# ACMEAtronOmatic/DSen2

Hardware: AMD Instinct MI355X
Metric: 32x32x6 patches/sec (DSen2_20, d=6, batch 512) (higher is better)
Workload: dtype f32; 1 GPU; DSen2_20 d=6 F=128 fp32, 512 synthetic 32x32 patches (4+6 bands) per GPU per step, he_uniform random-init weights; batch_per_gpu=512, parallelism=patch-sharded dp1, backend=rccl, output_gather=False

## Files before the change

dsen2_amd/asm_contract.py:

```python
import os
import re
import subprocess
import tempfile

HERE = os.path.dirname(os.path.abspath(__file__))
CSRC = os.path.join(HERE, 'csrc')
DMA_SOURCES = ['conv3x3_body32.hip', 'conv3x3_body16w.hip']


class AsmContractError(RuntimeError):
    pass


def _code_lines(text):
    return [ln.strip() for ln in text.splitlines() if ln.strip() and not ln.strip().startswith((';', '.', '//'))]


def _kernels(text):
    out, name, body = {}, None, []
    for ln in text.splitlines():
        m = re.match(r'^(_Z\w+):', ln)
        if m:
            name, body = m.group(1), []
            continue
# ... 6 lines not shown
                name = None
    return out


def normalised(body):
    return [re.sub(r'\.L\w+', 'L', re.sub(r'\s+', ' ', ln)) for ln in body]


def compile_isa(hipcc, flags, path, out, verbose=False):
    cmd = [hipcc] + [f for f in flags if f != '-fPIC'] + ['-S', '--cuda-device-only', path, '-o', out]
    if verbose:
        print(' '.join(cmd), flush=True)
    subprocess.check_call(cmd, stderr=subprocess.DEVNULL)
    with open(out) as f:
        return f.read()


def _needer(src):
    def need(cond, msg, ctx=()):
        if not cond:
            raise AsmContractError('%s: %s %s' % (src, msg, list(ctx)))
    return need


def check_listing(text, src):
    code = _code_lines(text)
    code = [ln.split(';')[0].strip() for ln in code]
    need = _needer(src)

    m0 = [i for i, ln in enumerate(code) if re.search(r'\bm0\b', ln)]
    need(m0, 'no M0 use found (the DMA statements are gone?)')
    dma = [i for i, ln in enumerate(code) if ln.startswith('buffer_load_dword') and ln.endswith('lds')]
    need(dma, 'no LDS-DMA instruction found')
    allowed = set()
    for i in dma:
        need(code[i - 1] == 's_nop 0' and re.match(r's_mov_b32 m0, (s\d+|vcc_lo|vcc_hi)$', code[i - 2]), 'DMA without its M0 write + wait state',
             code[i - 2:i + 1])
        allowed.update((i - 2,))
        for j in range(i - 3, max(i - 7, -1), -1):
            if re.match(r's_mov_b32 (s\d+|vcc_lo|vcc_hi), m0$', code[j]):
                allowed.add(j)
                break
        k = i + 1
        if re.match(r's_mov_b32 m0, (s\d+|vcc_lo|vcc_hi)$', code[k]):
            allowed.add(k)
    for i in m0:
        need(i in allowed, 'M0 touched outside a DMA statement', code[max(0, i - 2):i + 3])
    saves = sum(1 for ln in code if re.match(r's_mov_b32 (s\d+|vcc_lo|vcc_hi), m0$', ln))
    need(saves > 0, 'the DMA statements no longer save M0')
    STEP_MFMAS = 9 * 32
    need(not any(ln.startswith(('s_swappc', 's_call')) for ln in code), 'a DMA kernel calls a function (an epilogue was not inlined)')
    kernels = _kernels(text)
    need(kernels, 'no kernel found')
    n_dma_kernels = 0
    for name, body in kernels.items():
        if not any(ln.startswith('buffer_load_dword') and ln.endswith('lds') for ln in body):
            continue
        n_dma_kernels += 1
        chain = '_chain_kernel' in name
        if not chain:
            need(not any('scratch_' in ln for ln in body), 'kernel %s spills registers' % name)
        else:
            mf = [i for i, ln in enumerate(body) if ln.startswith('v_mfma')]
            need(mf and len(mf) % STEP_MFMAS == 0, 'chain kernel %s: %d MFMAs is not a whole number of item bodies' % (name, len(mf)))
            for g in range(0, len(mf), STEP_MFMAS):
                inner = body[mf[g]:mf[g + STEP_MFMAS - 1]]
                need(not any('scratch_' in ln for ln in inner), 'chain kernel %s spills inside an item body' % name)
            for i, ln in enumerate(body):
                if 'scratch_' not in ln:
                    continue
                nxt = None
                for ln2 in body[i + 1:]:
                    if ln2.startswith('v_mfma'):
                        break
                    mm = re.search(r'vmcnt\((\d+)\)', ln2) if ln2.startswith('s_waitcnt') else None
                    if mm:
                        nxt = int(mm.group(1))
                        break
                need(nxt == 0, 'chain kernel %s: scratch access outside a drained region (next vmcnt wait: %r)' % (name, nxt), [ln])
        back = [ln for ln in body[-40:] if ln.startswith('s_waitcnt') and 'vmcnt' in ln]
        need(back and back[-1].replace(' ', '') in ('s_waitcntvmcnt(0)', 's_waitcntvmcnt(0)lgkmcnt(0)'),
             'kernel %s does not drain its DMAs before s_endpgm' % name, back[-3:])
    need(n_dma_kernels > 0, 'no LDS-DMA kernel found')
    if src == 'conv3x3_body16w.hip':
        expect = {0: (0, 32), 1: (64, 64), 3: (64, 64)}
        expect3 = {0: (0, 64), 1: (64, 96), 3: (64, 64)}

        def count(pattern, want, msg, product=lambda m: True):
            found = []
            for name, body in kernels.items():
                m = re.search(pattern, name)
                if not m or not product(m):
                    continue
                found.append(body)
                loads = sum(1 for ln in body if ln.startswith('buffer_load_dwordx4') and not ln.endswith('lds'))
                stores = sum(1 for ln in body if ln.startswith('buffer_store_dwordx4'))
                need((loads, stores) == want(m), msg(m) % (loads, stores, want(m)))
            return found

        def total(e):
            return lambda m: (sum(v[0] for v in e.values()), sum(v[1] for v in e.values()))

        found = count(r'conv3x3_body16[wx]_kernelILi(\d+)ELi(\d+)ELi(\d+)ELi(\d+)E', lambda m: expect[int(m.group(3))],
                      lambda m: 'epilogue ' + m.group(3) + ' has %d loads / %d stores, the waits count %r', lambda m: int(m.group(4)) == 0)
        need(len(found) >= 6, 'expected the 6 product instantiations of the bf16 body kernel, found %d' % len(found))
        for body in found:
            other = [ln for ln in body if re.match(r'(buffer|global|flat)_(load|store|atomic)', ln)
                     and not ln.startswith(('buffer_load_dwordx4', 'buffer_store_dwordx4'))]
            need(len(other) <= 1, 'unexpected vector-memory instructions in the bf16 body kernel', other[:4])
        found3 = count(r'conv3x3_body16w_x3_kernelILi(\d+)ELi(\d+)ELi(\d+)E', lambda m: expect3[int(m.group(3))],
                       lambda m: 'bf16x3 epilogue ' + m.group(3) + ' has %d loads / %d stores, the waits count %r')
        need(len(found3) == 6, 'expected the 6 instantiations of the bf16x3 body kernel, found %d' % len(found3))
        chains = count(r'conv3x3_body16w_chain_kernelILi(\d+)ELi(\d+)ELi(\d+)E', total(expect),
                       lambda m: 'chain kernel has %d loads / %d stores in its epilogues, the waits count %r', lambda m: int(m.group(3)) == 0)
        need(len(chains) == 2, 'expected the 2 product instantiations of the chain kernel, found %d' % len(chains))
        chains3 = count(r'conv3x3_body16w_x3_chain_kernelILi(\d+)ELi(\d+)E', total(expect3),
                        lambda m: 'bf16x3 chain kernel has %d loads / %d stores in its epilogues, the waits count %r')
        need(len(chains3) == 2, 'expected the 2 instantiations of the bf16x3 chain kernel, found %d' % len(chains3))


def check_out_mfma_listing(text, src='conv3x3_out_mfma.hip'):
    need = _needer(src)
    kernels = {k: v for k, v in _kernels(text).items() if 'conv3x3_out_mfma_kernel' in k}
    need(len(kernels) == 4, 'expected 4 instantiations of the output kernel, found %d' % len(kernels))
    for name, body in kernels.items():
        need(not any('scratch_' in ln for ln in body), 'kernel %s spills registers' % name)
        need(not any(ln.startswith(('s_swappc', 's_call')) for ln in body), 'kernel %s calls a function' % name)
        mf = [i for i, ln in enumerate(body) if ln.startswith('v_mfma')]
        need(mf, 'kernel %s has no MFMA' % name)
        waits = [ln for ln in body[mf[0]:mf[-1]] if ln.startswith('s_waitcnt') and 'vmcnt' in ln]
        need(len(waits) >= 8, 'kernel %s: no operand waits between its MFMAs' % name)
        bad = [ln for ln in waits if int(re.search(r'vmcnt\((\d+)\)', ln).group(1)) < 8]
        need(not bad, 'kernel %s waits for the loads of the NEXT unit' % name, bad[:4])
    return True


def check_first16_listing(text, src='conv3x3_first16.hip'):
    need = _needer(src)
    kernels = {k: v for k, v in _kernels(text).items() if 'conv3x3_first16_kernel' in k}
    need(len(kernels) == 8, 'expected 8 instantiations of the kernel, found %d' % len(kernels))
    for name, body in kernels.items():
        need(not any('scratch_' in ln for ln in body), 'kernel %s spills registers' % name)
        need(not any(ln.startswith(('s_swappc', 's_call')) for ln in body), 'kernel %s calls a function' % name)
        stores = [ln for ln in body if ln.startswith('buffer_store_dwordx4')]
        need(stores, 'kernel %s has no 128-bit buffer store' % name)
        bad = [ln for ln in stores if not re.search(r'\], 0 offen', ln)]
        need(not bad, 'kernel %s: 128-bit buffer store with a register soffset (late data read, unpadded hazard)' % name, bad[:2])
        need(not any(ln.startswith('global_store') for ln in body), 'kernel %s stores outside its buffer descriptors' % name)
        mf = [i for i, ln in enumerate(body) if ln.startswith('v_mfma')]
        need(mf, 'kernel %s has no MFMA' % name)
        x3 = 'ELb1EEE' in name
        floor = 24 if x3 else 16
        loop = body[mf[0]:]
        scat = [i for i, ln in enumerate(loop) if ln.startswith('ds_write_b16')]
        need(scat, 'kernel %s: no halo scatter after the first MFMA' % name)
        waits = [ln for ln in loop[:scat[-1]] if ln.startswith('s_waitcnt') and 'vmcnt' in ln]
        low = [ln for ln in waits if int(re.search(r'vmcnt\((\d+)\)', ln).group(1)) < floor]
        need(not low, 'kernel %s: a wait inside the tile loop drains the deferred stores (divergent branch in the loop body?)' % name, low[:4])
    return True


TRAFFIC_KERNELS = {
    'dsen2_20_fp32': ('conv3x3_body32.hip', r'conv3x3_body32_kernelILi128ELi128ELi0ELi0ELi0ELb1ELb1E'),
    'vdsen2_20_bf16': ('conv3x3_body16w.hip', r'conv3x3_body16w_chain_kernelILi128ELi256ELi0E'),
    'dsen2_20_bf16x3': ('conv3x3_body16w.hip', r'conv3x3_body16w_x3_chain_kernelILi64ELi128E'),
    'vdsen2_20_fp32': ('conv3x3_body32.hip', r'conv3x3_body32_kernelILi256ELi256ELi0ELi0ELi0ELb1ELb1E'),
    'dsen2_20_bf16': ('conv3x3_body16w.hip', r'conv3x3_body16w_chain_kernelILi64ELi128ELi0E'),
    'vdsen2_20_bf16x3': ('conv3x3_body16w.hip', r'conv3x3_body16w_x3_chain_kernelILi128ELi256E'),
}
ISA_JSON = os.path.join(HERE, 'kernel_isa.json')


def isa_hashes(text):
    import hashlib
    out = {}
    for name, body in _kernels(text).items():
        out[name] = hashlib.sha256('\n'.join(normalised(body)).encode()).hexdigest()
    return out


def traffic_kernel_hashes(listings):
    out = {}
    for cfg, (src, pat) in TRAFFIC_KERNELS.items():
        hits = {k: v for k, v in isa_hashes(listings[src]).items() if re.search(pat, k)}
        if len(hits) != 1:
            raise AsmContractError('%s: expected one kernel matching %s, found %d' % (src, pat, len(hits)))
        (k, v), = hits.items()
        out[cfg] = {'kernel': k, 'isa_sha256': v}
    return out


def check_sources(hipcc, flags, verbose=False, isa_json=None):
    listings = {}
    with tempfile.TemporaryDirectory(prefix='dsen2_asm_') as tmp:
        for src in DMA_SOURCES + ['conv3x3_out_mfma.hip', 'conv3x3_first16.hip']:
            listings[src] = compile_isa(hipcc, flags, os.path.join(CSRC, src), os.path.join(tmp, src + '.s'), verbose)
            if src in DMA_SOURCES:
                check_listing(listings[src], src)
            elif src == 'conv3x3_first16.hip':
                check_first16_listing(listings[src], src)
            else:
                check_out_mfma_listing(listings[src], src)
    hashes = traffic_kernel_hashes(listings)
    if isa_json:
        import json
        with open(isa_json, 'w') as f:
            json.dump(hashes, f, indent=1, sort_keys=True)
            f.write('\n')
    return hashes
```

dsen2_amd/csrc/capi.hip:

```cpp

#include <chrono>
#include <cstdarg>
#include <cstdio>
#include <cstring>
#include <exception>
#include <new>
#include <vector>

#include "capi_internal.h"

using namespace dsen2;

namespace {

thread_local char g_err[512] = "";

#ifdef DSEN2_DIAG
Tuning g_diag_tuning;
unsigned long long* g_diag_stamps = nullptr;
#endif
Tuning default_tuning() {
#ifdef DSEN2_DIAG
  return g_diag_tuning;
#else
// ... 317 lines not shown
    off += align_up(floats);
    return p;
  };
  if (mask & ~1) {
    r.x10 = take(pix * m->c10);
    r.x20 = take(pix * m->c20);
    if (m->c60 > 0) r.x60 = take(pix * m->c60);
    r.y = take(pix * m->cout);
  }
  r.bytes = off * sizeof(float);
  return r;
}

static int check_ensemble_shape(const dsen2_model* m, int n, int h, int w, int mask) {
  if (mask <= 0 || mask > 255) return fail(DSEN2_ERR_INVALID, "ensemble mask %d outside 1..255", mask);
  if (int rc = check_shape(m, n, h, w)) return rc;
  if (int rc = check_shape(m, n, w, h)) return rc;
  int cmax = m->cout;
  for (int c : {m->c10, m->c20, m->c60}) cmax = c > cmax ? c : cmax;
  if ((size_t)n * h * w * cmax >= ((size_t)1 << 31))
    return fail(DSEN2_ERR_INVALID, "batch of %d images of %dx%d: a tensor of 2^31 elements or more", n, h, w);
  return DSEN2_OK;
}

static int forward_ensemble(dsen2_model* m, const float* x10, const float* x20, const float* x60, float* out, int n, int h, int w,
                            int mask, void* workspace, size_t workspace_bytes, void* stream_) {
  if (!m || !x10 || !x20 || !out || !workspace) return fail(DSEN2_ERR_INVALID, "NULL argument");
  if ((m->c60 > 0) != (x60 != nullptr)) return fail(DSEN2_ERR_INVALID, "x60 must be given iff the model has a 60 m input");
  if (mask <= 0 || mask > 255) return fail(DSEN2_ERR_INVALID, "ensemble mask %d outside 1..255", mask);
  if (n == 0) return DSEN2_OK;
  if (!m->loaded) return fail(DSEN2_ERR_NO_WEIGHTS, "dsen2_model_load_weights has not been called");
  if (int rc = check_ensemble_shape(m, n, h, w, mask)) return rc;
  if (int rc = check_device(m)) return rc;
  const size_t pix = (size_t)n * h * w;
  const float* const ins[3] = {x10, x20, x60};
  const int cs[3] = {m->c10, m->c20, m->c60};
  for (int k = 0; k < 3; ++k)
    if (ins[k] && overlaps(ins[k], pix * cs[k] * sizeof(float), out, pix * m->cout * sizeof(float)))
      return fail(DSEN2_ERR_INVALID, "the output aliases an input");
  const EnsembleWs E = ensemble_ws(m, n, h, w, mask, reinterpret_cast<char*>(workspace));
  if (workspace_bytes < E.bytes) return fail(DSEN2_ERR_WORKSPACE, "workspace %zu < %zu bytes", workspace_bytes, E.bytes);
  hipStream_t stream = (hipStream_t)stream_;
  int count = 0;
  for (int op = 0; op < 8; ++op) count += (mask >> op) & 1;
  int done = 0;
  for (int op = 0; op < 8; ++op) {
    if (!((mask >> op) & 1)) continue;
    const bool first = done == 0, last = done + 1 == count;
    if (op == 0) {
      const ForwardWs B = forward_ws(m, n, h, w, E.fwd);
      if (int rc = forward_launches(m, x10, x20, x60, out, n, h, w, B, 0, false, stream, nullptr)) return rc;
    } else {
      const bool tr = op & 1;
      const int th = tr ? w : h, tw = tr ? h : w;
      float* const turned[3] = {E.x10, E.x20, E.x60};
      for (int k = 0; k < 3; ++k)
        if (ins[k]) HIP_TRY(launch_dihedral(ins[k], turned[k], n, cs[k], h, w, op, nullptr, false, stream));
      const ForwardWs B = forward_ws(m, n, th, tw, E.fwd);
      if (int rc = forward_launches(m, E.x10, E.x20, E.x60, E.y, n, th, tw, B, 0, false, stream, nullptr)) return rc;
      if (first) HIP_TRY(launch_dihedral(E.y, out, n, m->cout, th, tw, op, nullptr, true, stream));
      else HIP_TRY(launch_dihedral_accumulate(E.y, out, n, m->cout, h, w, op, last ? count : 0, stream));
    }
    ++done;
  }
  return DSEN2_OK;
}

extern "C" {

const char* dsen2_version(void) {
#ifdef DSEN2_DIAG
  return "dsen2_hip 0.3-diag (gfx950; fp32 MFMA 32x32x2 / bf16 MFMA 16x16x32 / bf16x3; DIAGNOSTIC build)";
#else
  return "dsen2_hip 0.3 (gfx950; fp32 MFMA 32x32x2 / bf16 MFMA 16x16x32 / bf16x3)";
#endif
}
const char* dsen2_last_error(void) { return g_err; }

#ifdef DSEN2_DIAG
int dsen2_diag_set(int key, int value) {
  Tuning& t = g_diag_tuning;
  switch (key) {
    case 0:
      if (value != 0 && (value < 11 || value > 14)) return fail(DSEN2_ERR_INVALID, "body variant %d unknown", value);
      t.first = value == 0 ? FirstKernel::Tile16 : FirstKernel::Direct;
      t.body = value == 0 ? BodyKernel::Tile : BodyKernel::Body32;
      t.body32 = value == 0 ? Body32Form::DeferStagger : static_cast<Body32Form>(value - 11);
      return DSEN2_OK;
    case 2:
      if (value != 0 && value != 2 && value != 3) return fail(DSEN2_ERR_INVALID, "output variant %d unknown", value);
      t.out = value == 2 ? OutKernel::MfmaThenValu : value == 3 ? OutKernel::Valu : OutKernel::Tile;
      return DSEN2_OK;
    case 1: t.ablate = value; return DSEN2_OK;
    case 3: t.grid_cap = value; return DSEN2_OK;
    case 4: t.chain = value; return DSEN2_OK;
    case 5: t.first_ablate = value; return DSEN2_OK;
    case 6: t.out_ablate = value; return DSEN2_OK;
  }
  return fail(DSEN2_ERR_INVALID, "unknown diagnostic key %d", key);
}
int dsen2_diag_set_stamps(void* dev_buffer) {
  g_diag_stamps = reinterpret_cast<unsigned long long*>(dev_buffer);
  return DSEN2_OK;
}
#endif

int dsen2_device_count(void) {
  int n = 0;
  hipError_t e = hipGetDeviceCount(&n);
  if (e != hipSuccess) {
    (void)hipGetLastError();
    return fail(DSEN2_ERR_NO_DEVICE, "hipGetDeviceCount: %s", hipGetErrorString(e));
  }
  int good = 0;
  for (int i = 0; i < n; ++i) {
    hipDeviceProp_t prop;
    if (hipGetDeviceProperties(&prop, i) == hipSuccess && strncmp(prop.gcnArchName, "gfx950", 6) == 0) ++good;
  }
  return good;
}

int dsen2_model_create(dsen2_model** out, int c10, int c20, int c60, int num_layers, int feature_size, int precision) {
  return guarded([&]() -> int {
    if (!out) return fail(DSEN2_ERR_INVALID, "out is NULL");
    *out = nullptr;
    if (c10 <= 0 || c20 <= 0 || c60 < 0 || num_layers < 0) return fail(DSEN2_ERR_INVALID, "bad channel/layer counts");
    if (feature_size != 128 && feature_size != 256)
      return fail(DSEN2_ERR_INVALID, "feature_size %d unsupported (128 or 256)", feature_size);
    if (precision < 0 || precision > 2)
      return fail(DSEN2_ERR_INVALID, "precision %d unknown (0 = fp32, 1 = bf16 operands, 2 = bf16x3)", precision);
    const int cin = c10 + c20 + c60;
    const int cout = c60 > 0 ? c60 : c20;
    if (cin > 16) return fail(DSEN2_ERR_INVALID, "%d input channels > 16", cin);
    dsen2_model* m = new (std::nothrow) dsen2_model();
    if (!m) return fail(DSEN2_ERR_INVALID, "out of host memory");
    m->c10 = c10; m->c20 = c20; m->c60 = c60; m->cin = cin; m->cout = cout;
    m->num_layers = num_layers; m->feat = feature_size; m->precision = precision;
    m->dev_params = nullptr; m->loaded = false; m->train = nullptr;
    m->tune = default_tuning();
    if (hipGetDevice(&m->device) != hipSuccess) {
      delete m;
      return fail(DSEN2_ERR_NO_DEVICE, "no HIP device");
    }
    if (!plan_network(c10, c20, c60, num_layers, feature_size, precision, m->tune, m)) {
      delete m;
      return fail(DSEN2_ERR_INVALID, "no kernel for a layer of this network");
    }
    *out = m;
    return DSEN2_OK;
  });
}

void dsen2_model_destroy(dsen2_model* m) {
  if (!m) return;
  train_state_destroy(m->train);
  if (m->dev_params) (void)hipFree(m->dev_params);
  delete m;
}

size_t dsen2_model_num_params(const dsen2_model* m) { return m ? m->n_params : 0; }

int dsen2_model_load_weights(dsen2_model* m, const float* host_flat, size_t count) {
  return guarded([&]() -> int {
    if (!m || !host_flat) return fail(DSEN2_ERR_INVALID, "NULL argument");
    if (count != m->n_params)
      return fail(DSEN2_ERR_INVALID, "expected %zu parameters, got %zu", m->n_params, count);
    if (int rc = check_device(m)) return rc;
    std::vector<float> staged(m->dev_param_floats);
    for (const Layer& L : m->layers) {
      const float* k = host_flat + L.flat_off;
// ... 255 lines not shown
```

dsen2_amd/csrc/conv3x3_body32.hip:

```cpp
#include <type_traits>

#include "conv3x3_dma.h"

namespace dsen2 {

namespace {

using dma::KC; using dma::NT; using dma::THREADS; using dma::QS; using dma::IN_BYTES; using dma::IN_BLOCKS;
using dma::WCH; using dma::NWBUF; using dma::LDS_BYTES; using dma::wait_vmcnt;
constexpr int KSTEPS = 4;
constexpr int PB = 2, MB = 2;
static_assert((8 * kHalo) % 16 == 0, "rows R and R+8 of a pixel block sit on the same banks");

}

template <int CIN, int COUT, int EPI, int ABL, int PRE, bool STG, bool DEFER>
__global__ __launch_bounds__(THREADS, 2) void conv3x3_body32_kernel(const ConvParams p, const int n_items) {
  constexpr int NCC = CIN / KC;
  constexpr int NS = COUT / NT;
  static_assert(NCC % 2 == 0, "input double buffer parity");
  constexpr int N_W = (ABL & 4) ? 0 : 2;

  extern __shared__ __attribute__((aligned(16))) float smem[];
  float* const in_s = smem;
  float* const w_s = smem + 2 * IN_BYTES / 4;
  float* const bias_s = w_s + NWBUF * WCH;

  const int tid = threadIdx.x;
  const int lane = tid & 63;
  const int wave = __builtin_amdgcn_readfirstlane(tid >> 6);
  const int wn = wave & 1;
  const int wp = wave >> 1;
  const int l31 = lane & 31;
  const int hsel = lane >> 5;
  const int rh = l31 >> 4, c16 = l31 & 15;

  const int G = gridDim.x;
  const int lid = xcd_contiguous_id(blockIdx.x, G);
  if (lid >= n_items) return;
  const int my_items = (n_items - lid + G - 1) / G;
  const int tiles_per_img = p.tiles_x * p.tiles_y;
  const size_t img_pix = (size_t)p.h * p.w;

  dma::Stage<CIN, NS> st;
  st.init(p, in_s, w_s, lane, wave, lid, G, n_items);

  const int x_lane = (hsel * QS + (2 * wp + 8 * rh) * kHalo + c16) * 4;
  const int w_lane = (hsel * NT + wn * 64 + l31) * 4;

  st.set_stage_item(lid);
  if constexpr (!(ABL & 8)) {
#pragma unroll
    for (int b = 0; b < IN_BLOCKS; ++b) st.issue_in(0, b, 0);
  }
  if constexpr (!(ABL & 4)) {
    st.issue_w();
    st.issue_w();
    st.issue_w();
  }
  if (tid < COUT) bias_s[tid] = p.bias[tid];
  wait_vmcnt<0>();
  __syncthreads();

  f32x4 w_cur[MB], x_cur[PB], w_nxt[MB], x_nxt[PB];
  int mf_slot = 0;
  auto read_frags = [&](f32x4 (&wf)[MB], f32x4 (&xf)[PB], const float* ib, const float* wb, int tap, int s) {
    const int dy = tap / 3, dx = tap - dy * 3;
    const float* wp_ = wb + w_lane + (2 * s * NT) * 4;
    const float* xp_ = ib + x_lane + (2 * s * QS + dy * kHalo + dx) * 4;
#pragma unroll
    for (int mb = 0; mb < MB; ++mb) wf[mb] = *reinterpret_cast<const f32x4*>(wp_ + mb * 32 * 4);
#pragma unroll
    for (int pb = 0; pb < PB; ++pb) xf[pb] = *reinterpret_cast<const f32x4*>(xp_ + pb * kHalo * 4);
  };
  read_frags(w_cur, x_cur, in_s, w_s, 0, 0);

  struct OutGeom { int img; unsigned lane_eoff; int ey; bool col_ok; int chb; };
  auto out_geom = [&](int item, bool valid) -> OutGeom {
    const Tile t = tile_at<NS>(item, tiles_per_img, p.tiles_x);
    const int chb = t.slab * NT + wn * 64 + 4 * hsel;
    const int ex = t.tx0 + c16, ey = t.ty0 + 2 * wp + 8 * rh;
    return OutGeom{t.img, (unsigned)((ey * p.w + ex) * COUT + chb), ey, valid && ex < p.w, chb};
  };
  auto aux_desc = [&](int img) {
    return __builtin_amdgcn_make_buffer_rsrc(
        const_cast<float*>(p.aux) + (EPI == kEpiResidual ? (size_t)img * img_pix * COUT : 0), 0,
        EPI == kEpiResidual ? (unsigned)(img_pix * COUT * 4) : 0, 0x00020000);
  };
  auto byte_off = [&](const OutGeom& g_, int mb, int pb, int g) -> unsigned {
    return g_.col_ok && g_.ey + pb < p.h ? (g_.lane_eoff + (unsigned)(pb * p.w * COUT + mb * 32 + 8 * g)) * 4u : 0x80000000u;
  };

  auto run = [&](auto mid_c) {
  constexpr int MIDS = decltype(mid_c)::value;
  f32x16 acc[MB][PB];
#pragma unroll
  for (int mb = 0; mb < MB; ++mb)
#pragma unroll
    for (int pb = 0; pb < PB; ++pb)
#pragma unroll
      for (int e = 0; e < 16; ++e) acc[mb][pb][e] = 0.f;
  constexpr int kPre = EPI == kEpiResidual && !(ABL & 2) && !DEFER ? PRE : 0;
  f32x4 resv[kPre ? kPre : 1][PB][4];
#pragma unroll
  for (int mb = 0; mb < (kPre ? kPre : 1); ++mb)
#pragma unroll
    for (int pb = 0; pb < PB; ++pb)
#pragma unroll
      for (int g = 0; g < 4; ++g) resv[mb][pb][g] = f32x4{0.f, 0.f, 0.f, 0.f};

  f32x16 held[DEFER ? MB : 1][DEFER ? PB : 1];
  f32x4 rq[DEFER && EPI == kEpiResidual ? 4 : 1];
  for (int it = 0; it <= my_items; ++it) {
    const OutGeom g_ = out_geom(it > 0 ? lid + (it - 1) * G : lid, it > 0);
    const auto aux_rsrc = aux_desc(g_.img);
    const auto out_rsrc = __builtin_amdgcn_make_buffer_rsrc(
        p.out + (size_t)g_.img * img_pix * COUT, 0, (unsigned)(img_pix * COUT * 4), 0x00020000);
    auto load_res = [&](int j) -> f32x4 {
      const int mb = j >> 3, pb = (j >> 2) & 1, g = j & 3;
      return __builtin_bit_cast(f32x4, __builtin_amdgcn_raw_buffer_load_b128(aux_rsrc, byte_off(g_, mb, pb, g), 0, 0));
    };
    auto finish = [&](int j, const f32x16& a, f32x4 rr) {
      const int mb = j >> 3, pb = (j >> 2) & 1, g = j & 3;
      const f32x4 bias = *reinterpret_cast<const f32x4*>(bias_s + g_.chb + mb * 32 + 8 * g);
      f32x4 v = {a[4 * g], a[4 * g + 1], a[4 * g + 2], a[4 * g + 3]};
      v = v + bias;
      if constexpr (EPI == kEpiRelu) {
#pragma unroll
        for (int e = 0; e < 4; ++e) v[e] = fmaxf(v[e], 0.f);
      } else {
        v = rr + v * p.res_scale;
      }
      if constexpr (!(ABL & 1))
        __builtin_amdgcn_raw_buffer_store_b128(__builtin_bit_cast(u32x4, v), out_rsrc, byte_off(g_, mb, pb, g), 0, 0);
      else
        asm volatile("" ::"v"(v));
    };
    constexpr bool kRes = EPI == kEpiResidual && !(ABL & 2);
    if constexpr (!DEFER) {
#pragma unroll
      for (int j = 0; j < 16; ++j) {
        const int mb = j >> 3, pb = (j >> 2) & 1, g = j & 3;
        f32x4 rr = {1.f, 1.f, 1.f, 1.f};
        if constexpr (kRes) rr = mb < kPre ? resv[mb][pb][g] : load_res(j);
        finish(j, acc[mb][pb], rr);
      }
    } else {
#pragma unroll
      for (int mb = 0; mb < MB; ++mb)
#pragma unroll
        for (int pb = 0; pb < PB; ++pb) held[mb][pb] = acc[mb][pb];
      if (it == my_items) {
#pragma unroll
        for (int j = 0; j < 16; ++j) {
          f32x4 rr = {1.f, 1.f, 1.f, 1.f};
          if constexpr (kRes) rr = load_res(j);
          finish(j, held[j >> 3][(j >> 2) & 1], rr);
        }
      } else if constexpr (kRes) {
        rq[0] = load_res(0);
        rq[1] = load_res(1);
      }
    }
    if (it == my_items) break;
    const int item = lid + it * G;
    const bool have_next_item = it + 1 < my_items;
#pragma unroll
    for (int mb = 0; mb < MB; ++mb)
#pragma unroll
      for (int pb = 0; pb < PB; ++pb)
#pragma unroll
        for (int e = 0; e < 16; ++e) acc[mb][pb][e] = 0.f;

    auto do_cc = [&](const int cc, auto first_c) {
      constexpr bool kFirst = decltype(first_c)::value;
      (void)kFirst;
      const float* const ib = in_s + (cc & 1) * (IN_BYTES / 4);
      const float* const ib_next = in_s + ((cc + 1) & 1) * (IN_BYTES / 4);
      const bool last_cc = cc == NCC - 1;
      const int in_cc = last_cc ? 0 : cc + 1;
      if (last_cc && have_next_item) st.set_stage_item(item + G);
#pragma unroll
      for (int tap = 0; tap < 9; ++tap) {
        const float* const wb = w_s + mf_slot * WCH;
        const int nx_slot = mf_slot == NWBUF - 1 ? 0 : mf_slot + 1;
        const float* const wb_nx = w_s + nx_slot * WCH;
        constexpr int kNoIn = (ABL & 8) ? 1 : 0;
        const int n_in = (tap < IN_BLOCKS && !kNoIn) ? 1 : 0;

#pragma unroll
        for (int s = 0; s < KSTEPS; ++s) {
          if (s < KSTEPS - 1) {
            read_frags(w_nxt, x_nxt, ib, wb, tap, s + 1);
          } else if (tap < 8) {
            read_frags(w_nxt, x_nxt, ib, wb_nx, tap + 1, 0);
          } else {
            read_frags(w_nxt, x_nxt, ib_next, wb_nx, 0, 0);
          }
          if constexpr (DEFER) {
            if (kFirst && tap < 8) {
              if (s == MIDS && kRes && tap < 7) {
                rq[2 * ((tap + 1) & 1)] = load_res(2 * tap + 2);
                rq[2 * ((tap + 1) & 1) + 1] = load_res(2 * tap + 3);
              }
            }
          }
          if (s == MIDS) {
            if (n_in) st.issue_in((cc + 1) & 1, tap < IN_BLOCKS ? tap : 0, in_cc);
            if constexpr (!(ABL & 4)) st.issue_w();
          }
          if constexpr (DEFER) {
            if (kFirst && tap < 8 && (s == 1 || s == 3)) {
              const int j = 2 * tap + (s >> 1);
              f32x4 rr = {1.f, 1.f, 1.f, 1.f};
              if constexpr (kRes) rr = rq[2 * (tap & 1) + (s >> 1)];
              finish(j, held[j >> 3][(j >> 2) & 1], rr);
            }
          }
          if constexpr (kPre > 0 && !DEFER) {
            if (tap == 8 && last_cc && s == (MIDS < KSTEPS - 1 ? MIDS + 1 : MIDS)) {
              const OutGeom g_ = out_geom(item, true);
              const auto aux_rsrc = aux_desc(g_.img);
#pragma unroll
              for (int mb = 0; mb < kPre; ++mb)
#pragma unroll
                for (int pb = 0; pb < PB; ++pb)
#pragma unroll
                  for (int g = 0; g < 4; ++g)
                    resv[mb][pb][g] = __builtin_bit_cast(f32x4, __builtin_amdgcn_raw_buffer_load_b128(
                                                                    aux_rsrc, byte_off(g_, mb, pb, g), 0, 0));
            }
          }
          __builtin_amdgcn_sched_barrier(0);
#pragma unroll
          for (int j = 0; j < 4; ++j)
#pragma unroll
            for (int mb = 0; mb < MB; ++mb)
#pragma unroll
              for (int pb = 0; pb < PB; ++pb)
                acc[mb][pb] = __builtin_amdgcn_mfma_f32_32x32x2f32(w_cur[mb][j], x_cur[pb][j], acc[mb][pb], 0, 0, 0);
#pragma unroll
          for (int q = 0; q < MB; ++q) w_cur[q] = w_nxt[q];
#pragma unroll
          for (int q = 0; q < PB; ++q) x_cur[q] = x_nxt[q];
        }
        mf_slot = nx_slot;
        __builtin_amdgcn_sched_barrier(0);
        if (n_in) wait_vmcnt<N_W + 1>(); else wait_vmcnt<N_W>();
        if constexpr (!(ABL & 16)) __syncthreads();
      }
    };
    do_cc(0, std::true_type{});
#pragma unroll 1
    for (int cc = 1; cc < NCC; ++cc) do_cc(cc, std::false_type{});
  }
  };
  if constexpr (STG) {
    if (wave < 4)
      run(std::integral_constant<int, 0>{});
    else
      run(std::integral_constant<int, KSTEPS / 2>{});
  } else {
    run(std::integral_constant<int, 0>{});
  }
  wait_vmcnt<0>();
}

template <int CIN, int COUT, int EPI, int ABL = 0, int PRE = 0, bool STG = false, bool DEFER = false>
static hipError_t launch_body32_one(const ConvParams& p, hipStream_t stream) {
  const long long items = (long long)p.n * p.tiles_x * p.tiles_y * (COUT / NT);
  return launch_persistent<conv3x3_body32_kernel<CIN, COUT, EPI, ABL, PRE, STG, DEFER>>(LDS_BYTES, THREADS, items, 1, 0, stream, p);
}

template <int F>
static hipError_t launch_body32_feat(const ConvParams& p, int epilogue, Body32Form form, hipStream_t stream) {
  const bool relu = epilogue == kEpiRelu;
#ifdef DSEN2_DIAG
  if (form == Body32Form::Plain || form == Body32Form::StaggerA) {
    if (!relu) return launch_body32_one<F, F, kEpiResidual, 0, 2, false>(p, stream);
    return form == Body32Form::Plain ? launch_body32_one<F, F, kEpiRelu, 0, 0, false>(p, stream) : launch_body32_one<F, F, kEpiRelu, 0, 0, true>(p, stream);
  }
  if (form == Body32Form::DeferStaggerA && !relu) return launch_body32_one<F, F, kEpiResidual, 0, 0, false, true>(p, stream);
#else
  if (form != Body32Form::DeferStagger) return hipErrorInvalidValue;
#endif
  return relu ? launch_body32_one<F, F, kEpiRelu, 0, 0, true, true>(p, stream) : launch_body32_one<F, F, kEpiResidual, 0, 0, true, true>(p, stream);
}

hipError_t launch_conv3x3_body32(const ConvParams& p, int feat, int epilogue, Body32Form form, int ablate, hipStream_t stream) {
  if ((size_t)p.h * p.w * feat * 4 >= 0x80000000ull) return hipErrorNotSupported;
#ifdef DSEN2_DIAG
  if (feat == 128 && ablate != 0) {
#define DSEN2_ABL(M)                                                                             \
  if (ablate == M)                                                                               \
    return epilogue == kEpiRelu ? launch_body32_one<128, 128, kEpiRelu, M>(p, stream)            \
                                : launch_body32_one<128, 128, kEpiResidual, M, 2>(p, stream);
    DSEN2_ABL(1) DSEN2_ABL(2) DSEN2_ABL(3) DSEN2_ABL(4) DSEN2_ABL(8) DSEN2_ABL(12) DSEN2_ABL(15) DSEN2_ABL(16) DSEN2_ABL(31)
#undef DSEN2_ABL
    return hipErrorInvalidValue;
  }
#endif
  if (ablate != 0) return hipErrorInvalidValue;
  if (feat == 128) return launch_body32_feat<128>(p, epilogue, form, stream);
  if (feat == 256) return launch_body32_feat<256>(p, epilogue, form, stream);
  return hipErrorInvalidValue;
}

}
```

dsen2_amd/csrc/conv3x3_dma.h:

```cpp
#pragma once
#include "conv3x3_items.h"

namespace dsen2 {
namespace dma {

constexpr int KC = 32;
constexpr int NT = 128;
constexpr int THREADS = 512;
constexpr int QS = 336;
constexpr int IN_BYTES = 8 * QS * 16;
constexpr int IN_BLOCKS = 6;
constexpr int WCH = KC * NT;
constexpr int NWBUF = 4;
constexpr size_t LDS_BYTES = (size_t)2 * IN_BYTES + (size_t)NWBUF * WCH * 4 + 256 * 4;
static_assert(QS >= kHaloPix && QS % 16 == 0 && 64 * (IN_BLOCKS - 1) + 16 == QS, "input chunk geometry");
static_assert(LDS_BYTES <= 160 * 1024, "LDS budget");

template <int N>
__device__ __forceinline__ void wait_vmcnt() {
  static_assert(N >= 0 && N <= 63, "vmcnt is a 6-bit field");
  asm volatile("s_waitcnt vmcnt(%0)" ::"n"(N) : "memory");
}

__device__ __forceinline__ unsigned lds_address(const float* p) {
  return (unsigned)(size_t)(__attribute__((address_space(3))) const float*)p;
}

template <int CINW, int NS, bool LAZY_VOFF = false>
struct Stage {
  static constexpr int NCC = CINW / KC;
  static constexpr int NCHUNK = NCC * 9;

  const float* in;
  int h, w, tiles_x, tiles_per_img;
  size_t img_pix;
  int lane, wave, lid, G, n_items;
  unsigned lds_in, lds_w;
  unsigned in_voff[LAZY_VOFF ? 1 : IN_BLOCKS];
  int st_y0, st_x0;
  __amdgpu_buffer_rsrc_t in_rsrc, w_rsrc;
  unsigned w_voff;
  int wl_item, wl_chunk, st_slot;

  __device__ __forceinline__ void init(const ConvParams& p, const float* in_s, const float* w_s, int lane_, int wave_,
                                       int lid_, int G_, int n_items_) {
    in = p.in; h = p.h; w = p.w; tiles_x = p.tiles_x; tiles_per_img = p.tiles_x * p.tiles_y;
    img_pix = (size_t)p.h * p.w;
    lane = lane_; wave = wave_; lid = lid_; G = G_; n_items = n_items_;
    lds_in = lds_address(in_s);
    lds_w = lds_address(w_s);
    in_rsrc = __builtin_amdgcn_make_buffer_rsrc(const_cast<float*>(p.in), 0, 0, 0x00020000);
    w_rsrc = __builtin_amdgcn_make_buffer_rsrc(const_cast<float*>(p.wpk), 0, (unsigned)(NS * NCHUNK * WCH * 4), 0x00020000);
    w_voff = lane * 16;
    wl_item = lid; wl_chunk = 0; st_slot = 0;
    st_y0 = st_x0 = 0;
  }

  __device__ __forceinline__ unsigned voff_of(int b, int ty0, int tx0) const {
    const int hp = 64 * b + lane;
    const int hy = hp / kHalo, hx = hp - hy * kHalo;
    const int gy = ty0 - 1 + hy, gx = tx0 - 1 + hx;
    const bool inb = hp < kHaloPix && (unsigned)gy < (unsigned)h && (unsigned)gx < (unsigned)w;
    return inb ? (unsigned)(((gy * w + gx) * CINW + wave * 4) * 4) : 0x80000000u;
  }

  __device__ __forceinline__ void set_stage_item(int item) {
    const Tile t = tile_at<NS>(item, tiles_per_img, tiles_x);
    in_rsrc = __builtin_amdgcn_make_buffer_rsrc(const_cast<float*>(in) + (size_t)t.img * img_pix * CINW, 0,
                                                (unsigned)(img_pix * CINW * 4), 0x00020000);
    if constexpr (LAZY_VOFF) {
      st_y0 = t.ty0;
      st_x0 = t.tx0;
    } else {
#pragma unroll
      for (int b = 0; b < IN_BLOCKS; ++b) in_voff[b] = voff_of(b, t.ty0, t.tx0);
    }
  }

  __device__ __forceinline__ void issue_in(int buf, int b, int cc) {
    const unsigned m0v = lds_in + buf * IN_BYTES + (wave * QS + 64 * b) * 16;
    const unsigned so = cc * (KC * 4);
    const unsigned voff = LAZY_VOFF ? voff_of(b, st_y0, st_x0) : in_voff[LAZY_VOFF ? 0 : b];
    unsigned saved_m0;
    if (b < IN_BLOCKS - 1) {
      asm volatile("s_mov_b32 %0, m0\n\ts_mov_b32 m0, %1\n\ts_nop 0\n\tbuffer_load_dwordx4 %2, %3, %4 offen lds\n\ts_mov_b32 m0, %0"
                   : "=&s"(saved_m0) : "s"(m0v), "v"(voff), "s"(in_rsrc), "s"(so) : "memory");
    } else if (lane < 16) {
      asm volatile("s_mov_b32 %0, m0\n\ts_mov_b32 m0, %1\n\ts_nop 0\n\tbuffer_load_dwordx4 %2, %3, %4 offen lds\n\ts_mov_b32 m0, %0"
                   : "=&s"(saved_m0) : "s"(m0v), "v"(voff), "s"(in_rsrc), "s"(so) : "memory");
    }
  }

  __device__ __forceinline__ void issue_w() {
    const unsigned so = (unsigned)(((wl_item % NS) * NCHUNK + wl_chunk) * (WCH * 4) + wave * 1024);
    const unsigned l0 = lds_w + st_slot * (WCH * 4) + wave * 1024;
    unsigned saved_m0;
    asm volatile(
        "s_mov_b32 %0, m0\n\t"
        "s_mov_b32 m0, %1\n\ts_nop 0\n\tbuffer_load_dwordx4 %3, %4, %5 offen lds\n\t"
        "s_mov_b32 m0, %2\n\ts_nop 0\n\tbuffer_load_dwordx4 %3, %4, %6 offen lds\n\t"
        "s_mov_b32 m0, %0"
        : "=&s"(saved_m0) : "s"(l0), "s"(l0 + 8192u), "v"(w_voff), "s"(w_rsrc), "s"(so), "s"(so + 8192u)
        : "memory");
    if (++wl_chunk == NCHUNK) {
      wl_chunk = 0;
      wl_item = wl_item + G < n_items ? wl_item + G : lid;
    }
    st_slot = st_slot == NWBUF - 1 ? 0 : st_slot + 1;
  }
};

}
}
```

dsen2_amd/csrc/dsen2_internal.h:

```cpp
#pragma once
#include <hip/hip_runtime.h>
#include <stddef.h>
#include <stdint.h>

#include <mutex>

namespace dsen2 {


constexpr int kTile = 16;
constexpr int kHalo = kTile + 2;
constexpr int kHaloPix = kHalo * kHalo;

enum Epilogue : int {
  kEpiRelu = 0, kEpiResidual = 1, kEpiSkipNCHW = 2,
  kEpiResidualF32 = 3,
  kEpiReluSplit = 4
};

struct ConvParams {
  const float* in;
  const float* wpk;
  const float* bias;
  const float* aux;
  float* out;
  void* out2;
  int n, h, w;
  int tiles_x, tiles_y;
  int cout_real;
  float res_scale;
  unsigned long long* diag;
};

enum class FirstKernel { Direct, Tile16 };
enum class BodyKernel { Body32, Tile };
enum class Body32Form { StaggerA, Plain, DeferStaggerA, DeferStagger };
enum class OutKernel { MfmaThenValu, Valu, Tile };
struct Tuning {
  FirstKernel first = FirstKernel::Direct;
  BodyKernel body = BodyKernel::Body32;
  Body32Form body32 = Body32Form::DeferStagger;
  OutKernel out = OutKernel::MfmaThenValu;
  int ablate = 0;
  int grid_cap = 0;
  int first_ablate = 0;
  int out_ablate = 0;
  int chain = 1;
  static Tuning reference() { Tuning t; t.first = FirstKernel::Tile16; t.body = BodyKernel::Tile; t.out = OutKernel::Tile; return t; }
};

struct KernelOnce {
  std::mutex mu;
  bool done[64] = {};
  int cus[64] = {};
  hipError_t prepare(const void* kern, size_t lds_bytes, int* dev_cus) {
    int dev = 0;
    hipError_t e = hipGetDevice(&dev);
    if (e != hipSuccess) return e;
    if (dev < 0 || dev >= 64) return hipErrorInvalidDevice;
    std::lock_guard<std::mutex> lock(mu);
    if (!done[dev]) {
      if (lds_bytes > 0) {
        e = hipFuncSetAttribute(kern, hipFuncAttributeMaxDynamicSharedMemorySize, (int)lds_bytes);
        if (e != hipSuccess) return e;
      }
      e = hipDeviceGetAttribute(&cus[dev], hipDeviceAttributeMultiprocessorCount, dev);
      if (e != hipSuccess) return e;
      done[dev] = true;
    }
    if (dev_cus) *dev_cus = cus[dev];
    return hipSuccess;
  }
};

hipError_t launch_conv3x3_tile(const ConvParams& p, int cin_pad, int cout_pad, int epilogue, int real_channels, hipStream_t stream);
hipError_t launch_conv3x3_out_valu(const ConvParams& p, int feat, hipStream_t stream);
void pack_out_valu_weights_host(const float* kernel_hwio, int cin, int cout, float* dst);
hipError_t launch_conv3x3_out_mfma(const ConvParams& p, int feat, hipStream_t stream, int ablate = 0);
size_t out_mfma_weight_floats(int cin);
void pack_out_mfma_weights_host(const float* kernel_hwio, int cin, int cout, float* dst);
struct FirstInputs { const float* x60; int c10, c20, c60; };
hipError_t launch_conv3x3_first(const ConvParams& p, const FirstInputs& f, int cout, int epilogue, hipStream_t stream, int ablate = 0);
hipError_t launch_conv3x3_first16(const ConvParams& p, const FirstInputs& f, int cout, bool x3, hipStream_t stream);
size_t first16_weight_u16(int cout, bool x3);
void pack_first16_weights_host(const float* kernel_hwio, int cin, int cout, bool x3, uint16_t* dst);
hipError_t launch_conv3x3_body32(const ConvParams& p, int feat, int epilogue, Body32Form form, int ablate, hipStream_t stream);
hipError_t launch_conv3x3_body16w(const ConvParams& p, int feat, int epilogue, bool x3, int ablate, hipStream_t stream, int grid_cap = 0);
hipError_t launch_split3_f32(const float* in_nhwc, void* hx, void* lo, int n, int h, int w, int c, hipStream_t stream);
struct ChainArgs {
  void* hi;
  void* lo;
  void* t;
  float* out_f32;
  unsigned layer_stride;
  int n_layers;
  int patches_per_wg;
  int seamless;
};
hipError_t launch_conv3x3_body16w_chain(const ConvParams& p, const ChainArgs& c, int feat, hipStream_t stream, int ablate = 0,
                                        bool x3 = false);
int body16w_chain_patches_per_wg(int n, int h, int w, int feat, int cus);
hipError_t launch_split_f32(const float* in_nhwc, void* hi, void* lo, int n, int h, int w, int c, hipStream_t stream);
hipError_t launch_join_f32(const void* hi, const void* lo, float* out_nhwc, int n, int h, int w, int c, hipStream_t stream);
inline uint16_t f32_to_bf16_rne(float f) {
  uint32_t u = __builtin_bit_cast(uint32_t, f);
  if ((u & 0x7fffffffu) > 0x7f800000u) return (uint16_t)((u >> 16) | 0x40);
  u += 0x7fffu + ((u >> 16) & 1u);
  return (uint16_t)(u >> 16);
}

hipError_t launch_pack_inputs(const float* x10, const float* x20, const float* x60, int c10, int c20, int c60,
                              float* out_nhwc16, int n, int h, int w, hipStream_t stream);
hipError_t launch_upsample(const float* in, float* out, int planes, int h, int w, int oh, int ow, float post_div,
                           hipStream_t stream, bool general = false);
hipError_t launch_tile_gather(const float* img, int H, int W, int C, int border, const int* origins, int count,
                              int P, float divisor, float* patches, hipStream_t stream);
hipError_t launch_recompose(const float* patches, int count, int C, int P, int border, float* img, int H, int W,
                            float scale, int row0, int row1, hipStream_t stream);

hipError_t launch_dihedral(const float* in, float* out, int n, int c, int ih, int iw, int op, const int* dev_ops, bool inverse,
                           hipStream_t stream);
hipError_t launch_dihedral_accumulate(const float* in, float* acc, int n, int c, int h, int w, int op, int count, hipStream_t stream);
__host__ __device__ __forceinline__ int dihedral_bits(int op) {
  return (int)(0x72416350u >> (4 * (op & 7))) & 7;
// ... 57 lines not shown
```

Measured before the change: 40150 patches/s.

## Make fp32 body conv waves asymmetric: half issue all LDS DMAs, half compute only

Adds a DeferAsym form of the fp32 body conv kernel and makes it the default. Waves 0-3 now issue every input and weight LDS-DMA load at twice the per-statement count, and waves 4-7 run a compute-only copy of the item loop with no M0 manipulation or vmcnt waits. The aim is to take DMA issue and wait overhead off half the waves so their MFMA stream runs uninterrupted. In exchange the issuing waves carry more DMA work and longer waits, which could make them the critical path. The asm contract checks are extended to verify the two loop copies.

Result: faster. 40570 patches/s (median of 6 runs) (+1.0%).

```diff
diff --git a/dsen2_amd/asm_contract.py b/dsen2_amd/asm_contract.py
--- a/dsen2_amd/asm_contract.py
+++ b/dsen2_amd/asm_contract.py
@@ -112,6 +112,29 @@
         need(back and back[-1].replace(' ', '') in ('s_waitcntvmcnt(0)', 's_waitcntvmcnt(0)lgkmcnt(0)'),
              'kernel %s does not drain its DMAs before s_endpgm' % name, back[-3:])
     need(n_dma_kernels > 0, 'no LDS-DMA kernel found')
+    if src == 'conv3x3_body32.hip':
+        ITEM_MFMAS = 2 * 9 * 64
+        asym = {k: v for k, v in kernels.items() if re.search(r'conv3x3_body32_kernelILi\d+ELi\d+ELi\d+ELi\d+ELi\d+ELi[2-9]E', k)}
+        need(asym, 'no DeferAsym instantiation of the fp32 body kernel found')
+        for name, body in asym.items():
+            mf = [i for i, ln in enumerate(body) if ln.startswith('v_mfma')]
+            need(len(mf) == 2 * ITEM_MFMAS, 'kernel %s: %d MFMAs, expected two copies of the item loop' % (name, len(mf)))
+            copies = [body[mf[0]:mf[ITEM_MFMAS - 1]], body[mf[ITEM_MFMAS]:mf[-1]]]
+            n_dma = [sum(1 for ln in c if ln.startswith('buffer_load_dword') and ln.endswith('lds')) for c in copies]
+            need(min(n_dma) == 0 and max(n_dma) > 0, 'kernel %s: DMAs in both copies of the item loop' % name, n_dma)
+            quiet, loud = (copies[0], copies[1]) if n_dma[0] == 0 else (copies[1], copies[0])
+            need(not any(re.search(r'\bm0\b', ln) for ln in quiet), 'kernel %s: M0 use in the compute-only copy' % name)
+            run = None
+            for ln in loud:
+                if re.match(r's_mov_b32 (s\d+|vcc_lo|vcc_hi), m0$', ln):
+                    need(run is None, 'kernel %s: M0 saved twice in one DMA statement' % name)
+                    run = 0
+                elif ln.startswith('buffer_load_dword') and ln.endswith('lds'):
+                    need(run is not None, 'kernel %s: DMA outside a statement that saves M0' % name)
+                    run += 1
+                elif run and not re.match(r'(s_mov_b32 m0, |s_nop 0$)', ln):
+                    need(run in (2, 4), 'kernel %s: a DMA statement of %d instructions' % (name, run))
+                    run = None
     if src == 'conv3x3_body16w.hip':
         expect = {0: (0, 32), 1: (64, 64), 3: (64, 64)}
         expect3 = {0: (0, 64), 1: (64, 96), 3: (64, 64)}
@@ -191,10 +214,10 @@
 
 
 TRAFFIC_KERNELS = {
-    'dsen2_20_fp32': ('conv3x3_body32.hip', r'conv3x3_body32_kernelILi128ELi128ELi0ELi0ELi0ELb1ELb1E'),
+    'dsen2_20_fp32': ('conv3x3_body32.hip', r'conv3x3_body32_kernelILi128ELi128ELi0ELi0ELi0ELi4ELb1E'),
     'vdsen2_20_bf16': ('conv3x3_body16w.hip', r'conv3x3_body16w_chain_kernelILi128ELi256ELi0E'),
     'dsen2_20_bf16x3': ('conv3x3_body16w.hip', r'conv3x3_body16w_x3_chain_kernelILi64ELi128E'),
-    'vdsen2_20_fp32': ('conv3x3_body32.hip', r'conv3x3_body32_kernelILi256ELi256ELi0ELi0ELi0ELb1ELb1E'),
+    'vdsen2_20_fp32': ('conv3x3_body32.hip', r'conv3x3_body32_kernelILi256ELi256ELi0ELi0ELi0ELi4ELb1E'),
     'dsen2_20_bf16': ('conv3x3_body16w.hip', r'conv3x3_body16w_chain_kernelILi64ELi128ELi0E'),
     'vdsen2_20_bf16x3': ('conv3x3_body16w.hip', r'conv3x3_body16w_x3_chain_kernelILi128ELi256E'),
 }
diff --git a/dsen2_amd/csrc/capi.hip b/dsen2_amd/csrc/capi.hip
--- a/dsen2_amd/csrc/capi.hip
+++ b/dsen2_amd/csrc/capi.hip
@@ -423,10 +423,10 @@
   Tuning& t = g_diag_tuning;
   switch (key) {
     case 0:
-      if (value != 0 && (value < 11 || value > 14)) return fail(DSEN2_ERR_INVALID, "body variant %d unknown", value);
+      if (value != 0 && (value < 11 || value > 19)) return fail(DSEN2_ERR_INVALID, "body variant %d unknown", value);
       t.first = value == 0 ? FirstKernel::Tile16 : FirstKernel::Direct;
       t.body = value == 0 ? BodyKernel::Tile : BodyKernel::Body32;
-      t.body32 = value == 0 ? Body32Form::DeferStagger : static_cast<Body32Form>(value - 11);
+      t.body32 = value == 0 ? Body32Form::DeferAsym : static_cast<Body32Form>(value - 11);
       return DSEN2_OK;
     case 2:
       if (value != 0 && value != 2 && value != 3) return fail(DSEN2_ERR_INVALID, "output variant %d unknown", value);
diff --git a/dsen2_amd/csrc/conv3x3_body32.hip b/dsen2_amd/csrc/conv3x3_body32.hip
--- a/dsen2_amd/csrc/conv3x3_body32.hip
+++ b/dsen2_amd/csrc/conv3x3_body32.hip
@@ -14,12 +14,14 @@
 
 }
 
-template <int CIN, int COUT, int EPI, int ABL, int PRE, bool STG, bool DEFER>
+template <int CIN, int COUT, int EPI, int ABL, int PRE, int STG, bool DEFER>
 __global__ __launch_bounds__(THREADS, 2) void conv3x3_body32_kernel(const ConvParams p, const int n_items) {
   constexpr int NCC = CIN / KC;
   constexpr int NS = COUT / NT;
   static_assert(NCC % 2 == 0, "input double buffer parity");
-  constexpr int N_W = (ABL & 4) ? 0 : 2;
+  constexpr bool ASYM = STG >= 2;
+  using Stage = dma::Stage<CIN, NS, false, ASYM ? dma::Role::Issuer : dma::Role::All>;
+  constexpr int N_W = (ABL & 4) ? 0 : Stage::N_W;
 
   extern __shared__ __attribute__((aligned(16))) float smem[];
   float* const in_s = smem;
@@ -42,21 +44,23 @@
   const int tiles_per_img = p.tiles_x * p.tiles_y;
   const size_t img_pix = (size_t)p.h * p.w;
 
-  dma::Stage<CIN, NS> st;
+  Stage st;
   st.init(p, in_s, w_s, lane, wave, lid, G, n_items);
 
   const int x_lane = (hsel * QS + (2 * wp + 8 * rh) * kHalo + c16) * 4;
   const int w_lane = (hsel * NT + wn * 64 + l31) * 4;
 
-  st.set_stage_item(lid);
-  if constexpr (!(ABL & 8)) {
-#pragma unroll
-    for (int b = 0; b < IN_BLOCKS; ++b) st.issue_in(0, b, 0);
-  }
-  if constexpr (!(ABL & 4)) {
-    st.issue_w();
-    st.issue_w();
-    st.issue_w();
+  if (!ASYM || wave < 4) {
+    st.set_stage_item(lid);
+    if constexpr (!(ABL & 8)) {
+#pragma unroll
+      for (int b = 0; b < IN_BLOCKS; ++b) st.issue_in(0, b, 0);
+    }
+    if constexpr (!(ABL & 4)) {
+      st.issue_w();
+      st.issue_w();
+      st.issue_w();
+    }
   }
   if (tid < COUT) bias_s[tid] = p.bias[tid];
   wait_vmcnt<0>();
@@ -91,8 +95,9 @@
     return g_.col_ok && g_.ey + pb < p.h ? (g_.lane_eoff + (unsigned)(pb * p.w * COUT + mb * 32 + 8 * g)) * 4u : 0x80000000u;
   };
 
-  auto run = [&](auto mid_c) {
+  auto run = [&](auto mid_c, auto issue_c) {
   constexpr int MIDS = decltype(mid_c)::value;
+  constexpr bool ISSUE = decltype(issue_c)::value;
   f32x16 acc[MB][PB];
 #pragma unroll
   for (int mb = 0; mb < MB; ++mb)
@@ -179,14 +184,16 @@
       const float* const ib_next = in_s + ((cc + 1) & 1) * (IN_BYTES / 4);
       const bool last_cc = cc == NCC - 1;
       const int in_cc = last_cc ? 0 : cc + 1;
-      if (last_cc && have_next_item) st.set_stage_item(item + G);
+      if constexpr (ISSUE) {
+        if (last_cc && have_next_item) st.set_stage_item(item + G);
+      }
 #pragma unroll
       for (int tap = 0; tap < 9; ++tap) {
         const float* const wb = w_s + mf_slot * WCH;
         const int nx_slot = mf_slot == NWBUF - 1 ? 0 : mf_slot + 1;
         const float* const wb_nx = w_s + nx_slot * WCH;
         constexpr int kNoIn = (ABL & 8) ? 1 : 0;
-        const int n_in = (tap < IN_BLOCKS && !kNoIn) ? 1 : 0;
+        const int n_in = (tap < IN_BLOCKS && !kNoIn) ? Stage::N_IN : 0;
 
 #pragma unroll
         for (int s = 0; s < KSTEPS; ++s) {
@@ -205,9 +212,11 @@
               }
             }
           }
-          if (s == MIDS) {
-            if (n_in) st.issue_in((cc + 1) & 1, tap < IN_BLOCKS ? tap : 0, in_cc);
-            if constexpr (!(ABL & 4)) st.issue_w();
+          if constexpr (ISSUE) {
+            if (s == MIDS) {
+              if (n_in) st.issue_in((cc + 1) & 1, tap < IN_BLOCKS ? tap : 0, in_cc);
+              if constexpr (!(ABL & 4)) st.issue_w();
+            }
           }
           if constexpr (DEFER) {
             if (kFirst && tap < 8 && (s == 1 || s == 3)) {
@@ -246,7 +255,9 @@
         }
         mf_slot = nx_slot;
         __builtin_amdgcn_sched_barrier(0);
-        if (n_in) wait_vmcnt<N_W + 1>(); else wait_vmcnt<N_W>();
+        if constexpr (ISSUE) {
+          if (n_in) wait_vmcnt<N_W + Stage::N_IN>(); else wait_vmcnt<N_W>();
+        }
         if constexpr (!(ABL & 16)) __syncthreads();
       }
     };
@@ -255,42 +266,64 @@
     for (int cc = 1; cc < NCC; ++cc) do_cc(cc, std::false_type{});
   }
   };
-  if constexpr (STG) {
+  if constexpr (ASYM) {
+    if (wave < 4) {
+      run(std::integral_constant<int, (STG - 2) % KSTEPS>{}, std::true_type{});
+    } else {
+      if constexpr ((STG - 2) / KSTEPS == 1) __builtin_amdgcn_s_setprio(1);
+      run(std::integral_constant<int, 0>{}, std::false_type{});
+    }
+  } else if constexpr (STG == 1) {
     if (wave < 4)
-      run(std::integral_constant<int, 0>{});
+      run(std::integral_constant<int, 0>{}, std::true_type{});
     else
-      run(std::integral_constant<int, KSTEPS / 2>{});
+      run(std::integral_constant<int, KSTEPS / 2>{}, std::true_type{});
   } else {
-    run(std::integral_constant<int, 0>{});
+    run(std::integral_constant<int, 0>{}, std::true_type{});
   }
   wait_vmcnt<0>();
 }
 
-template <int CIN, int COUT, int EPI, int ABL = 0, int PRE = 0, bool STG = false, bool DEFER = false>
+template <int CIN, int COUT, int EPI, int ABL = 0, int PRE = 0, int STG = 0, bool DEFER = false>
 static hipError_t launch_body32_one(const ConvParams& p, hipStream_t stream) {
   const long long items = (long long)p.n * p.tiles_x * p.tiles_y * (COUT / NT);
   return launch_persistent<conv3x3_body32_kernel<CIN, COUT, EPI, ABL, PRE, STG, DEFER>>(LDS_BYTES, THREADS, items, 1, 0, stream, p);
 }
+
+constexpr int kAsym = 2 + KSTEPS / 2;
 
 template <int F>
 static hipError_t launch_body32_feat(const ConvParams& p, int epilogue, Body32Form form, hipStream_t stream) {
   const bool relu = epilogue == kEpiRelu;
 #ifdef DSEN2_DIAG
   if (form == Body32Form::Plain || form == Body32Form::StaggerA) {
-    if (!relu) return launch_body32_one<F, F, kEpiResidual, 0, 2, false>(p, stream);
-    return form == Body32Form::Plain ? launch_body32_one<F, F, kEpiRelu, 0, 0, false>(p, stream) : launch_body32_one<F, F, kEpiRelu, 0, 0, true>(p, stream);
-  }
-  if (form == Body32Form::DeferStaggerA && !relu) return launch_body32_one<F, F, kEpiResidual, 0, 0, false, true>(p, stream);
+    if (!relu) return launch_body32_one<F, F, kEpiResidual, 0, 2, 0>(p, stream);
+    return form == Body32Form::Plain ? launch_body32_one<F, F, kEpiRelu, 0, 0, 0>(p, stream) : launch_body32_one<F, F, kEpiRelu, 0, 0, 1>(p, stream);
+  }
+  if (form == Body32Form::DeferStaggerA && !relu) return launch_body32_one<F, F, kEpiResidual, 0, 0, 0, true>(p, stream);
+  if (form == Body32Form::DeferStagger || form == Body32Form::DeferStaggerA)
+    return relu ? launch_body32_one<F, F, kEpiRelu, 0, 0, 1, true>(p, stream) : launch_body32_one<F, F, kEpiResidual, 0, 0, 1, true>(p, stream);
+#define DSEN2_ASYM(FORM, STG)                                                                                      \
+  if (form == Body32Form::FORM)                                                                                    \
+    return relu ? launch_body32_one<F, F, kEpiRelu, 0, 0, STG, true>(p, stream) : launch_body32_one<F, F, kEpiResidual, 0, 0, STG, true>(p, stream);
+  DSEN2_ASYM(DeferAsymS0, 2) DSEN2_ASYM(DeferAsymS1, 3) DSEN2_ASYM(DeferAsymS3, 5) DSEN2_ASYM(DeferAsymPrio, 8)
+#undef DSEN2_ASYM
 #else
-  if (form != Body32Form::DeferStagger) return hipErrorInvalidValue;
+  if (form != Body32Form::DeferAsym) return hipErrorInvalidValue;
 #endif
-  return relu ? launch_body32_one<F, F, kEpiRelu, 0, 0, true, true>(p, stream) : launch_body32_one<F, F, kEpiResidual, 0, 0, true, true>(p, stream);
+  return relu ? launch_body32_one<F, F, kEpiRelu, 0, 0, kAsym, true>(p, stream) : launch_body32_one<F, F, kEpiResidual, 0, 0, kAsym, true>(p, stream);
 }
 
 hipError_t launch_conv3x3_body32(const ConvParams& p, int feat, int epilogue, Body32Form form, int ablate, hipStream_t stream) {
   if ((size_t)p.h * p.w * feat * 4 >= 0x80000000ull) return hipErrorNotSupported;
 #ifdef DSEN2_DIAG
   if (feat == 128 && ablate != 0) {
+#define DSEN2_ABL_ASYM(M)                                                                                \
+  if (ablate == M && form == Body32Form::DeferAsym)                                                      \
+    return epilogue == kEpiRelu ? launch_body32_one<128, 128, kEpiRelu, M, 0, kAsym, true>(p, stream)    \
+                                : launch_body32_one<128, 128, kEpiResidual, M, 0, kAsym, true>(p, stream);
+    DSEN2_ABL_ASYM(3) DSEN2_ABL_ASYM(15) DSEN2_ABL_ASYM(16)
+#undef DSEN2_ABL_ASYM
 #define DSEN2_ABL(M)                                                                             \
   if (ablate == M)                                                                               \
     return epilogue == kEpiRelu ? launch_body32_one<128, 128, kEpiRelu, M>(p, stream)            \
diff --git a/dsen2_amd/csrc/conv3x3_dma.h b/dsen2_amd/csrc/conv3x3_dma.h
--- a/dsen2_amd/csrc/conv3x3_dma.h
+++ b/dsen2_amd/csrc/conv3x3_dma.h
@@ -26,8 +26,12 @@
   return (unsigned)(size_t)(__attribute__((address_space(3))) const float*)p;
 }
 
-template <int CINW, int NS, bool LAZY_VOFF = false>
+enum class Role { All, Issuer };
+
+template <int CINW, int NS, bool LAZY_VOFF = false, Role ROLE = Role::All>
 struct Stage {
+  static constexpr int N_W = ROLE == Role::Issuer ? 4 : 2;
+  static constexpr int N_IN = ROLE == Role::Issuer ? 2 : 1;
   static constexpr int NCC = CINW / KC;
   static constexpr int NCHUNK = NCC * 9;
 
@@ -81,6 +85,24 @@
     const unsigned m0v = lds_in + buf * IN_BYTES + (wave * QS + 64 * b) * 16;
     const unsigned so = cc * (KC * 4);
     const unsigned voff = LAZY_VOFF ? voff_of(b, st_y0, st_x0) : in_voff[LAZY_VOFF ? 0 : b];
+    if constexpr (ROLE == Role::Issuer) {
+      const unsigned m1v = m0v + 4 * QS * 16, so1 = so + 64;
+      unsigned saved_m0;
+      if (b < IN_BLOCKS - 1) {
+        asm volatile("s_mov_b32 %0, m0\n\t"
+                     "s_mov_b32 m0, %1\n\ts_nop 0\n\tbuffer_load_dwordx4 %3, %4, %5 offen lds\n\t"
+                     "s_mov_b32 m0, %2\n\ts_nop 0\n\tbuffer_load_dwordx4 %3, %4, %6 offen lds\n\t"
+                     "s_mov_b32 m0, %0"
+                     : "=&s"(saved_m0) : "s"(m0v), "s"(m1v), "v"(voff), "s"(in_rsrc), "s"(so), "s"(so1) : "memory");
+      } else if (lane < 16) {
+        asm volatile("s_mov_b32 %0, m0\n\t"
+                     "s_mov_b32 m0, %1\n\ts_nop 0\n\tbuffer_load_dwordx4 %3, %4, %5 offen lds\n\t"
+                     "s_mov_b32 m0, %2\n\ts_nop 0\n\tbuffer_load_dwordx4 %3, %4, %6 offen lds\n\t"
+                     "s_mov_b32 m0, %0"
+                     : "=&s"(saved_m0) : "s"(m0v), "s"(m1v), "v"(voff), "s"(in_rsrc), "s"(so), "s"(so1) : "memory");
+      }
+      return;
+    }
     unsigned saved_m0;
     if (b < IN_BLOCKS - 1) {
       asm volatile("s_mov_b32 %0, m0\n\ts_mov_b32 m0, %1\n\ts_nop 0\n\tbuffer_load_dwordx4 %2, %3, %4 offen lds\n\ts_mov_b32 m0, %0"
@@ -95,6 +117,19 @@
     const unsigned so = (unsigned)(((wl_item % NS) * NCHUNK + wl_chunk) * (WCH * 4) + wave * 1024);
     const unsigned l0 = lds_w + st_slot * (WCH * 4) + wave * 1024;
     unsigned saved_m0;
+    if constexpr (ROLE == Role::Issuer)
+      asm volatile(
+          "s_mov_b32 %0, m0\n\t"
+          "s_mov_b32 m0, %1\n\ts_nop 0\n\tbuffer_load_dwordx4 %5, %6, %7 offen lds\n\t"
+          "s_mov_b32 m0, %2\n\ts_nop 0\n\tbuffer_load_dwordx4 %5, %6, %8 offen lds\n\t"
+          "s_mov_b32 m0, %3\n\ts_nop 0\n\tbuffer_load_dwordx4 %5, %6, %9 offen lds\n\t"
+          "s_mov_b32 m0, %4\n\ts_nop 0\n\tbuffer_load_dwordx4 %5, %6, %10 offen lds\n\t"
+          "s_mov_b32 m0, %0"
+          : "=&s"(saved_m0)
+          : "s"(l0), "s"(l0 + 4096u), "s"(l0 + 8192u), "s"(l0 + 12288u), "v"(w_voff), "s"(w_rsrc), "s"(so), "s"(so + 4096u),
+            "s"(so + 8192u), "s"(so + 12288u)
+          : "memory");
+    else
     asm volatile(
         "s_mov_b32 %0, m0\n\t"
         "s_mov_b32 m0, %1\n\ts_nop 0\n\tbuffer_load_dwordx4 %3, %4, %5 offen lds\n\t"
diff --git a/dsen2_amd/csrc/dsen2_internal.h b/dsen2_amd/csrc/dsen2_internal.h
--- a/dsen2_amd/csrc/dsen2_internal.h
+++ b/dsen2_amd/csrc/dsen2_internal.h
@@ -34,12 +34,12 @@
 
 enum class FirstKernel { Direct, Tile16 };
 enum class BodyKernel { Body32, Tile };
-enum class Body32Form { StaggerA, Plain, DeferStaggerA, DeferStagger };
+enum class Body32Form { StaggerA, Plain, DeferStaggerA, DeferStagger, DeferAsym, DeferAsymS0, DeferAsymS1, DeferAsymS3, DeferAsymPrio };
 enum class OutKernel { MfmaThenValu, Valu, Tile };
 struct Tuning {
   FirstKernel first = FirstKernel::Direct;
   BodyKernel body = BodyKernel::Body32;
-  Body32Form body32 = Body32Form::DeferStagger;
+  Body32Form body32 = Body32Form::DeferAsym;
   OutKernel out = OutKernel::MfmaThenValu;
   int ablate = 0;
   int grid_cap = 0;
```
